# PolyU-IOR/HPR-LP-C

Hardware: AMD Instinct MI355X
Metric: HPR iterations/sec (FP64) (higher is better)
Workload: dtype f64

## Files before the change

### hpr-lp-c_amd/csrc/abi.cpp

```cpp
#include <algorithm>
#include <cmath>
#include <cstdlib>
#include <cstring>
#include <memory>
#include <mutex>
#include <iomanip>
#include <iostream>

#include "hprlp_amd.h"
#include "batch_prep.h"
#include "batched.h"
#include "env.h"
#include "dist.h"
#include "presolve.h"
#include "reorder.h"
#include "solver.h"
#include "many.h"
#include "values.h"
#include "version.h"

using namespace hprlp;

struct hprlp_solver {
    Solver s;
// ... 1242 lines not shown
    if (name == "x_temp") return {s.x_temp, s.n_loc, 'c'};
    if (name == "y") return {s.y, s.m_loc, 'r'};
    if (name == "last_y") return {s.last_y.p, s.m_loc, 'r'};
    if (name == "y_bar") return {s.y_bar, s.m_loc, 'r'};
    if (name == "y_obj") return {s.y_obj.p, s.m_loc, 'r'};
    if (name == "y_temp") return {s.y_temp.p, s.m_loc, 'r'};
    if (name == "AL") return {s.AL.p, s.m_loc, 'r'};
    if (name == "AU") return {s.AU.p, s.m_loc, 'r'};
    if (name == "l") return {s.l.p, s.n_loc, 'c'};
    if (name == "u") return {s.u.p, s.n_loc, 'c'};
    if (name == "c") return {s.c.p, s.n_loc, 'c'};
    if (name == "row_norm") return {s.row_norm.p, s.m_loc, 'r'};
    if (name == "col_norm") return {s.col_norm.p, s.n_loc, 'c'};
    if (name == "A_val") return {s.A.val.p, s.A.view.nnz, '-'};
    if (name == "AT_val") return {s.AT.val.p, s.AT.view.nnz, '-'};
    return {nullptr, -1, '-'};
}
const std::vector<int> *perm_of(const Solver &s, const VecRef &v) {
    if (v.kind == 'r' && !s.perm_r.empty()) return &s.perm_r;
    if (v.kind == 'c' && !s.perm_c.empty()) return &s.perm_c;
    return nullptr;
}
}

extern "C" long hprlp_solver_get_vector(hprlp_solver *h, const char *name, double *out, long cap) {
    GUARD_BEGIN
    VecRef v = find_vector(h->s, name ? name : "");
    if (v.n < 0) throw std::runtime_error(std::string("unknown vector name: ") + (name ? name : "(null)"));
    if (cap < v.n) throw std::runtime_error("output buffer too small");
    HIP_CHECK(hipStreamSynchronize(h->s.stream));
// ... 312 lines not shown
        d += t.n_pieces > 0 ? "tiled, piece form (k_tiled_part + k_tiled_finish, " + std::to_string(t.n_pieces) + " pieces)"
             : t.rem_cap == kPbRemCap ? "tiled, all-remainder form (k_pb_fused, grid " + std::to_string(t.grid) + ")"
                                      : "tiled, fused (k_tiled_fused, grid " + std::to_string(t.grid) + ")";
        d += ", " + std::to_string(t.nsb) + " super-blocks, " + std::to_string(M.tiled.n_steps) + " steps";
        if (t.R != kTileRows || t.T != kTileCols) d += " (" + std::to_string(t.R) + " rows, tiles of " + std::to_string(t.T) + " columns)";
        const double all = static_cast<double>(M.tiled.dense_entries) + static_cast<double>(M.tiled.n_rem);
        if (all > 0) d += ", " + std::to_string(static_cast<int>(100.0 * M.tiled.dense_entries / all + 0.5)) + " % of the entries in staged tiles";
        if (t.f_rk) d += ", source-side run tables";
        if (t.f_work) d += ", pre-pass work list of " + std::to_string(t.n_work) + " workgroups for " + std::to_string(t.n_groups) + " source groups";
        if (t.side_nblk > 0) d += ", long rows aside (" + std::to_string(t.side_nblk) + " blocks through the stream kernel)";
        return d;
    };
    std::string d = one("A", s.A) + "; " + one("A^T", s.AT);
    if (s.use_small && !s.comm) d += "; normal iterations in the single-workgroup kernel (k_small_iterations)";
    if (!s.perm_r.empty()) d += "; locality ordering applied at set-up";
    if (!s.env_at_setup.empty()) d += "; switches: " + s.env_at_setup;
    if (!s.env_ignored_at_setup.empty()) d += "; ignored without HPRLP_TEST_HOOKS=1: " + s.env_ignored_at_setup;
    std::snprintf(buf, static_cast<size_t>(cap), "%s", d.c_str());
    return static_cast<int>(d.size());
    GUARD_END(-1)
}

extern "C" int hprlp_form_select(const hprlp_form_facts *facts, const hprlp_form_hooks *hooks, hprlp_form_decision *out) {
    try {
        if (!facts || !out) throw std::runtime_error("bad arguments");
        const char *missing = "";
        if (!form_select(*facts, hooks ? *hooks : FormHooks(), out, &missing))
            throw std::runtime_error(std::string("the rules ask for a fact that the record marks as not measured: ") + missing);
        return 0;
    } catch (const std::exception &e) {
// ... 103 lines not shown
```

### hpr-lp-c_amd/csrc/env.cpp

```cpp
#include "env.h"

#include <cstdlib>
#include <cstring>
#include <stdexcept>

namespace hprlp {

static const EnvEntry kTable[] = {
    {"HPRLP_TEST_HOOKS", EnvKind::Integrator, "1: honour the test hooks below (tests/conftest.py and the tools/ scripts set it)"},
    {"HPRLP_TIMING", EnvKind::Integrator, "wall time of the set-up and solve phases on stderr"},
    {"HPRLP_NO_GRAPH", EnvKind::Integrator, "launch normal iterations eagerly instead of replaying hipGraphs (fall-back)"},
    {"HPRLP_NO_TILED", EnvKind::Integrator, "never build the column-tiled matrix copies: stream kernel everywhere (fall-back)"},
    {"HPRLP_NO_REORDER", EnvKind::Integrator, "no set-up time locality ordering of a large matrix"},
    {"HPRLP_NO_ALLOC_CACHE", EnvKind::Integrator, "do not keep freed device blocks for the next solver of the process"},
    {"HPRLP_DIST_TRANSPORT", EnvKind::Integrator, "shm: hprlp_dist_unique_id names a shared-memory segment (host-staged group of processes on one node) instead of RCCL ids"},
    {"HPRLP_NO_WARM_MODEL", EnvKind::Integrator, "the model constructors do NOT start the HIP runtime / device context / code objects (for a process that forks workers after building its models: a HIP context does not survive fork); the first solve pays for them as in the reference"},
    {"HPRLP_DIST_EXCHANGE", EnvKind::Hook, "sparse | allgather: force the multi-GPU exchange form (same value on every rank)"},
    {"HPRLP_NO_OVERLAP", EnvKind::Integrator, "multi-GPU: shards unsplit, exchange in line on the solver stream"},
    {"HPRLP_DIST_TIMEOUT_S", EnvKind::Integrator, "seconds a rank of the shared-memory transport waits for its peers before it fails (default 120)"},
    {"HPRLP_BATCH_CHUNK", EnvKind::Hook, "solve_batched with 64 or more problems: chunk width of the panels (default 64; narrower chunks map one chunk to each XCD -- measured slower, profiles/r03_tiled_decomposition.md section 6b)"},
    {"HPRLP_BATCH_GRID", EnvKind::Hook, "solve_batched: cap on the row blocks of the normal half-step kernels (read at every call; a small cap makes every workgroup's row loop wrap)"},
    {"HPRLP_BATCH_LAMBDA", EnvKind::Hook, "solve_batched: the batch's lambda_max from the caller (strtod; hand it over as a C99 hex float to keep every bit) instead of 1.01 x the power iteration's estimate (read at every call)"},
    {"HPRLP_COPY_PAUSE_US", EnvKind::Hook, "piece size and pause of the threaded copies of set-up (64 MB, 100 us)"},
    {"HPRLP_COPY_PIECE_MB", EnvKind::Hook, "piece size and pause of the threaded copies of set-up (64 MB, 100 us)"},
// ... 7 lines not shown
    {"HPRLP_HOST_TRANSPOSE", EnvKind::Hook, "build Aᵀ on the host / nonzero threshold of the device transpose (default 4 M)"},
    {"HPRLP_NO_BOUND_CODES", EnvKind::Hook, "the x-half always reads l[j] and u[j], the y-half AL[i] and AU[i] (default: one code byte per column / row says which of them is not a constant; an equality row reads one value)"},
    {"HPRLP_NO_FAR_PUSH", EnvKind::Hook, "always run the remainder pre-pass (k_far_products) instead of the hand-off from the producing half-step's epilogue"},
    {"HPRLP_NO_FAR_WORK", EnvKind::Hook, "the remainder pre-pass with one workgroup per source group also where one group holds several times the mean (default: a work list cuts heavy groups into chunks, tiled.h f_work)"},
    {"HPRLP_NO_PB_LONG_ROWS", EnvKind::Hook, "a matrix kept off the tiled forms for its long rows keeps the stream kernel also where its columns are not popular (default: all-remainder form, Solver::pb_fallback_wanted)"},
    {"HPRLP_NO_FUSED_NORMS", EnvKind::Hook, "the Ruiz row norms by their own passes instead of as a by-product of the preceding scaling pass (same bits)"},
    {"HPRLP_NO_LONG_SIDE", EnvKind::Hook, "a matrix with rows over 1024 entries keeps the stream kernel instead of being tiled with those rows kept aside"},
    {"HPRLP_NO_PB_FALLBACK", EnvKind::Hook, "unstructured large matrices keep the stream kernel instead of the tiled form without dense-tile requirement"},
    {"HPRLP_NO_PB_KERNEL", EnvKind::Hook, "run an all-remainder copy through k_tiled_fused's remainder steps instead of k_pb_fused (A/B)"},
    {"HPRLP_NO_REM2", EnvKind::Hook, "tiled build: no second remainder level"},
    {"HPRLP_NO_SETUP_OVERLAP", EnvKind::Hook, "set-up of a large model in line: no helper threads / copy streams for the value upload, the row blocks, A^T's row pointers and the model vectors (same bits either way)"},
    {"HPRLP_NO_SLAB_CUTS", EnvKind::Hook, "dense rows of a large matrix are not cut at the XCD eighths of the gathered vector (stream kernel)"},
    {"HPRLP_NO_SMALL", EnvKind::Hook, "do not use the single-workgroup kernel for Netlib-scale LPs"},
    {"HPRLP_NO_SMALL_POWER", EnvKind::Hook, "Netlib-scale LPs: power iteration by the regular kernels with the host test every 10th iteration (default: one launch of the single-workgroup kernel)"},
    {"HPRLP_NO_TILED_CR", EnvKind::Hook, "Curtis-Reid passes through the stream kernel also for matrices with a tiled copy (default: tiled kernel on a second value array of -log|a|)"},
    {"HPRLP_NT", EnvKind::Hook, "force default / nontemporal loads of the matrix in the stream kernel"},
    {"HPRLP_OVERLAP_COMM_FIRST", EnvKind::Hook, "tests only: with the in-process rank group, use RCCL's launch order (exchange enqueued before the local SpMV)"},
    {"HPRLP_PB_MIN_COLS", EnvKind::Hook, "gathered-vector length from which an unstructured matrix takes the all-remainder form (default 800 k columns, the crossover measured with k_pb_fused)"},
    {"HPRLP_PB_MIN_NNZ", EnvKind::Hook, "fewest entries for the all-remainder form"},
    {"HPRLP_PB_STAMPS", EnvKind::Hook, "developer build -DHPRLP_PB_PHASE_STAMPS=1: print k_pb_fused's phase times"},
    {"HPRLP_PIECES_ANYWAY", EnvKind::Hook, "attempt the tiled form although neighbouring rows gather from the same lines (<= 0.25 lines per entry) / keep the piece form although an XCD's rows gather from under 3 MB"},
    {"HPRLP_PRESOLVE_MAX_LINKS", EnvKind::Hook, "run one presolve stage alone / cut the chain after n links (tests, debugging)"},
    {"HPRLP_PRESOLVE_OFF", EnvKind::Hook, "switch presolve reductions / stages off (any subset; diagnostics)"},
    {"HPRLP_PRESOLVE_ONLY", EnvKind::Hook, "run one presolve stage alone / cut the chain after n links (tests, debugging)"},
    {"HPRLP_REORDER_CLUSTER", EnvKind::Hook, "knobs of the HOST reference path of the ordering (hprlp_locality_ordering): nodes per cluster, refinement sweeps, trimming percentage"},
    {"HPRLP_REORDER_HOST", EnvKind::Hook, "run the clustering of the locality ordering on the host (the reference form; default: on the device)"},
    {"HPRLP_REORDER_SWEEPS", EnvKind::Hook, "knobs of the HOST reference path of the ordering (hprlp_locality_ordering): nodes per cluster, refinement sweeps, trimming percentage"},
    {"HPRLP_REORDER_TRIM", EnvKind::Hook, "knobs of the HOST reference path of the ordering (hprlp_locality_ordering): nodes per cluster, refinement sweeps, trimming percentage"},
    {"HPRLP_SLACK_PIVOT", EnvKind::Hook, "pivot threshold of the costed slack-column substitution (default 0.5 of the row's largest entry)"},
    {"HPRLP_STORE_X", EnvKind::Hook, "every normal x-half reads and stores x (default for matrices with a tiled copy: inside a run of normal iterations x is rebuilt from x_hat and last_x by the next launch instead of travelling through memory)"},
// ... 52 lines not shown
```

### hpr-lp-c_amd/csrc/kernels.hip

```cpp
#include "kernels.h"

#include <algorithm>
#include <vector>
#include <cmath>
#include <type_traits>

namespace hprlp {

__device__ __forceinline__ double wave_sum(double v) {
#pragma unroll
    for (int off = 32; off > 0; off >>= 1) v += __shfl_xor(v, off, kWave);
    return v;
}

__device__ __forceinline__ double wave_max(double v) {
#pragma unroll
    for (int off = 32; off > 0; off >>= 1) v = fmax(v, __shfl_xor(v, off, kWave));
    return v;
}

template <int NACC, int NW, int NMAX = 0>
__device__ __forceinline__ void block_store_partials_in(double (&acc)[NACC], double *partials, int stride, double (*red)[NACC > 0 ? NACC : 1]) {
    const int wave = threadIdx.x >> 6, lane = threadIdx.x & 63;
#pragma unroll
// ... 210 lines not shown
    const int v = q == 0 ? a0 : (q == 1 ? a1 : (q == 2 ? a2 : a3));
    return __builtin_amdgcn_readlane(v, r & 63);
}

#ifndef HPRLP_PB_PHASE_STAMPS
#define HPRLP_PB_PHASE_STAMPS 0
#endif
#ifndef HPRLP_SWEEP_ED
#define HPRLP_SWEEP_ED 2
#define HPRLP_SWEEP_TD 1
#endif
#ifndef HPRLP_EPI_NT
#define HPRLP_EPI_NT 2
#endif

template <int ED, int TD, bool REP, bool STAMP = false, bool LOGTERM = false, int TC = kTileCols>
__device__ __forceinline__ void tiled_sweep(const TiledDev &t, int s0, int nst, int first, int count, const double *__restrict__ vec,
                                            int ncols, double *acc, double *ytile, int tid, unsigned long long *stamp = nullptr) {
    constexpr int NT = kTileThreads, R = kTileRows, K = kTileChunk;
    constexpr int TPT = TC / NT;
    static_assert(TC == kTileCols || TC == kTileColsNarrow, "tile width");
    typedef double d2_t __attribute__((ext_vector_type(2)));
    const int lane = tid & 63;
    auto sidx = [&](int i) { i = min(i, count - 1) + first; return s0 + (i < nst ? i : i - nst); };
    int seg = 0, lim = 0;
    int tc0 = 0, tc1 = 0, tc2 = 0, tc3 = 0, tb0 = 0, tb1 = 0, tb2 = 0, tb3 = 0, te0 = 0, te1 = 0, te2 = 0, te3 = 0;
    auto getstep = [&](int k, int &col0, int &eb, int &ee) {
        const int r = min(k, lim - 1) - seg;
        col0 = step_field(tc0, tc1, tc2, tc3, r);
        eb = step_field(tb0, tb1, tb2, tb3, r);
        ee = step_field(te0, te1, te2, te3, r);
    };
    struct Ent {
// ... 39 lines not shown
    };
    auto process = [&](const Ent &E, int k) {
        int col0, eb, ee_;
        getstep(k, col0, eb, ee_);
        if (K * tid < ee_ - eb) {
            const double v[K] = {E.va.x, E.va.y, E.vb.x, E.vb.y};
            const uint32_t c0 = E.i0, c1 = E.i1, c2 = E.i2;
            const uint32_t id[K] = {c0 & 0xffffffu, (c0 >> 24) | ((c1 & 0xffffu) << 8), (c1 >> 16) | ((c2 & 0xffu) << 16), c2 >> 8};
            uint32_t rw[K];
            double y[K];
#pragma unroll
            for (int k2 = 0; k2 < K; ++k2) {
                rw[k2] = id[k2] & (R - 1);
                y[k2] = ytile[id[k2] >> kTileRowBits];
            }
            double a[K];
#pragma unroll
            for (int k2 = 0; k2 < K; ++k2) a[k2] = acc[rw[k2]];
            double sk[K], pr[K];
#pragma unroll
            for (int k2 = 0; k2 < K; ++k2) pr[k2] = LOGTERM ? (v[k2] != v[k2] ? 0.0 : v[k2] - y[k2]) : v[k2] * y[k2];
            sk[0] = a[0] + pr[0];
#pragma unroll
            for (int k2 = 1; k2 < K; ++k2) sk[k2] = ((rw[k2] == rw[k2 - 1]) ? sk[k2 - 1] : a[k2]) + pr[k2];
#pragma unroll
            for (int k2 = 0; k2 < K; ++k2)
                if (k2 == K - 1 || rw[k2] != rw[k2 + 1]) acc[rw[k2]] = sk[k2];
        }
    };
    auto same_tile = [&](int k) {
// ... 1788 lines not shown
                         bool divide, hipStream_t s, double *next_max_norm) {
    if (M.rows <= 0 || M.nblk <= 0) return;
    if (next_max_norm) {
        if (row_first && divide) launch_scale_matrix_t<true, true, true>(M, rowvec, colvec_full, next_max_norm, s);
        else if (row_first && !divide) launch_scale_matrix_t<true, false, true>(M, rowvec, colvec_full, next_max_norm, s);
        else if (!row_first && divide) launch_scale_matrix_t<false, true, true>(M, rowvec, colvec_full, next_max_norm, s);
        else launch_scale_matrix_t<false, false, true>(M, rowvec, colvec_full, next_max_norm, s);
        return;
    }
    if (row_first && divide) launch_scale_matrix_t<true, true, false>(M, rowvec, colvec_full, nullptr, s);
    else if (row_first && !divide) launch_scale_matrix_t<true, false, false>(M, rowvec, colvec_full, nullptr, s);
    else if (!row_first && divide) launch_scale_matrix_t<false, true, false>(M, rowvec, colvec_full, nullptr, s);
    else launch_scale_matrix_t<false, false, false>(M, rowvec, colvec_full, nullptr, s);
}

__global__ void __launch_bounds__(kThreads) k_vec_scale(double *x, const double *s, int n, int divide) {
    const int i = blockIdx.x * kThreads + threadIdx.x;
    if (i < n) x[i] = divide ? x[i] / s[i] : x[i] * s[i];
}
void launch_vec_scale(double *x, const double *sv, int n, bool divide, hipStream_t s) {
    if (n <= 0) return;
    hipLaunchKernelGGL(k_vec_scale, dim3((n + kThreads - 1) / kThreads), dim3(kThreads), 0, s, x, sv, n, divide ? 1 : 0);
}

__global__ void __launch_bounds__(kThreads) k_vec_scal(double *x, double a, int n) {
    const int i = blockIdx.x * kThreads + threadIdx.x;
    if (i < n) x[i] = x[i] * a;
}
void launch_vec_scal(double *x, double a, int n, hipStream_t s) {
    if (n <= 0) return;
// ... 322 lines not shown
```

### hpr-lp-c_amd/csrc/solver.cpp

```cpp
#include "solver.h"
#include "env.h"

#include <algorithm>
#include <cmath>
#include <cstdio>
#include <cstdlib>
#include <cstring>
#include <functional>
#include <iomanip>
#include <iostream>
#include <limits>
#include <thread>

#include "dist.h"
#include "reorder.h"

namespace hprlp {

constexpr int kMaxGraphIters = 64;
constexpr int kDeviceStartRows = 1000000;
constexpr int kPowerBlockKey = -10;

struct RowCuts {
    std::vector<int> rows;
// ... 1097 lines not shown
        gsm2.alloc(static_cast<size_t>(m_pad));
        gsn2.alloc(static_cast<size_t>(n_pad));
        HIP_CHECK(hipMemsetAsync(gsm2.p, 0, sizeof(double) * m_pad, stream));
        HIP_CHECK(hipMemsetAsync(gsn2.p, 0, sizeof(double) * n_pad, stream));
    }
    double *gm = gsm.p, *gn = gsn.p, *gm_next = gsm2.p, *gn_next = gsn2.p;
    double *t1 = gm + row_off, *t2 = gn + col_off;
    double *t1n = fuse_norms ? gm_next + row_off : nullptr, *t2n = fuse_norms ? gn_next + col_off : nullptr;
    bool have_norms = false;
    const bool max_next = fuse_norms;
    launch_fill(row_norm.p, 1.0, m_loc, stream);
    launch_fill(col_norm.p, 1.0, n_loc, stream);
    norm_b_org = 1.0 + std::sqrt(bnorm_sq(this));
    norm_c_org = 1.0 + std::sqrt(reduce_sum_sq(c.p, n_loc));

    if (prm.use_CR_scaling) {
        HIP_CHECK(hipMemsetAsync(gsm.p, 0, sizeof(double) * m_pad, stream));
        HIP_CHECK(hipMemsetAsync(gsn.p, 0, sizeof(double) * n_pad, stream));
        finish_tiling();
        struct LogValues {
            DBuf<double> tile, far;
        } logA, logAT;
        const bool tiled_cr = env_get("HPRLP_NO_TILED_CR") == nullptr;
        auto log_values = [&](DeviceMatrix &M, LogValues &lv) {
            if (!tiled_cr || !cr_runs_tiled(M.view)) return;
            lv.tile.alloc(static_cast<size_t>(std::max<long>(M.tiled.n_tile, 1)));
            lv.far.alloc(static_cast<size_t>(std::max<long>(M.tiled.n_rem, 1)));
            launch_tiled_refresh_log(M.tiled, M.val.p, lv.tile.p, lv.far.p, stream);
        };
        log_values(A, logA);
        log_values(AT, logAT);
        for (int it = 0; it < 20; ++it) {
            launch_cr_log_update(A.view, gsn.p, t1, stream, logA.tile.p, logA.far.p);
            gather(gsm.p, true);
            launch_cr_log_update(AT.view, gsm.p, t2, stream, logAT.tile.p, logAT.far.p);
            gather(gsn.p, false);
        }
        if (logA.tile.p || logAT.tile.p) HIP_CHECK(hipStreamSynchronize(stream));
        launch_exp_clamp(t1, m_loc, stream);
        launch_exp_clamp(t2, n_loc, stream);
        gather(gsm.p, true);
        gather(gsn.p, false);
        launch_vec_scale(row_norm.p, t1, m_loc, true, stream);
        launch_vec_scale(col_norm.p, t2, n_loc, true, stream);
        launch_scale_matrix(A.view, t1, gsn.p, true, false, stream, max_next ? t1n : nullptr);
        launch_scale_matrix(AT.view, t2, gsm.p, false, false, stream, max_next ? t2n : nullptr);
        have_norms = max_next;
        launch_vec_scale(AL.p, t1, m_loc, false, stream);
        launch_vec_scale(AU.p, t1, m_loc, false, stream);
        launch_vec_scale(c.p, t2, n_loc, false, stream);
        launch_vec_scale(l.p, t2, n_loc, true, stream);
        launch_vec_scale(u.p, t2, n_loc, true, stream);
    }

    const int passes = (prm.use_Ruiz_scaling ? 10 : 0) + (prm.use_Pock_Chambolle_scaling ? 1 : 0);
    for (int it = 0; it < passes; ++it) {
        const int norm = (prm.use_Ruiz_scaling && it < 10) ? 99 : 1;
        if (have_norms) {
            std::swap(gm, gm_next);
            std::swap(gn, gn_next);
            t1 = gm + row_off, t2 = gn + col_off, t1n = gm_next + row_off, t2n = gn_next + col_off;
        } else {
            launch_row_norm(A.view, t1, norm, stream);
            launch_row_norm(AT.view, t2, norm, stream);
        }
        gather(gm, true);
        gather(gn, false);
        launch_vec_scale(row_norm.p, t1, m_loc, false, stream);
        launch_vec_scale(AL.p, t1, m_loc, true, stream);
        launch_vec_scale(AU.p, t1, m_loc, true, stream);
        launch_vec_scale(col_norm.p, t2, n_loc, false, stream);
        const bool next = fuse_norms && it + 1 < passes && it + 1 < 10;
        launch_scale_matrix(A.view, t1, gn, true, true, stream, next ? t1n : nullptr);
        launch_scale_matrix(AT.view, t2, gm, false, true, stream, next ? t2n : nullptr);
        have_norms = next;
        launch_vec_scale(c.p, t2, n_loc, true, stream);
        launch_vec_scale(l.p, t2, n_loc, false, stream);
        launch_vec_scale(u.p, t2, n_loc, false, stream);
    }

    if (prm.use_bc_scaling) {
        b_scale = 1.0 + std::sqrt(bnorm_sq(this));
        c_scale = 1.0 + std::sqrt(reduce_sum_sq(c.p, n_loc));
        const double bs = 1.0 / b_scale, cs = 1.0 / c_scale;
        launch_vec_scal(AU.p, bs, m_loc, stream);
        launch_vec_scal(AL.p, bs, m_loc, stream);
        launch_vec_scal(l.p, bs, n_loc, stream);
        launch_vec_scal(u.p, bs, n_loc, stream);
        launch_vec_scal(c.p, cs, n_loc, stream);
    } else {
        b_scale = 1.0;
        c_scale = 1.0;
    }
    norm_b = std::sqrt(bnorm_sq(this));
    norm_c = std::sqrt(reduce_sum_sq(c.p, n_loc));
    finish_tiling();
    A.refresh_tiled(stream);
    AT.refresh_tiled(stream);
    refresh_bound_codes();
    HIP_CHECK(hipMemsetAsync(gsm.p, 0, sizeof(double) * m_pad, stream));
    HIP_CHECK(hipMemsetAsync(gsn.p, 0, sizeof(double) * n_pad, stream));
    HIP_CHECK(hipStreamSynchronize(stream));
    scaling_time = time_since(t0);
    scaled = true;
}

SmallArgs Solver::small_args() const {
    return SmallArgs{m, n, A.view.nnz, A.view.rowptr, AT.view.rowptr, AT.view.val, small_ij.p, small_posA.p,
                     small_order_x.p, small_order_y.p, x.p, x_hat, y, l.p, u.p, c.p, last_x.p, AL.p, AU.p, last_y.p, ctrl.p};
}

bool Solver::small_power_wanted() const {
    const bool no_small_power = env_get("HPRLP_NO_SMALL_POWER") != nullptr;
    return use_small && !comm && !no_small_power;
}

void Solver::power_start(double *z) {
// ... 801 lines not shown
```

### hpr-lp-c_amd/csrc/solver.h

```cpp
#pragma once

#include <string>
#include <vector>

#include <functional>
#include <future>
#include <map>
#include <memory>

#include "common.h"
#include "env.h"
#include "dist.h"
#include "kernels.h"
#include "hpr_rules.h"
#include "form_select.h"

namespace hprlp {

struct TraceRow {
    int iter, restart_flag;
    double err_Rp, err_Rd, primal_obj, dual_obj, gap, kkt, sigma, current_gap, lambda_max;
};

struct DeviceMatrix {
// ... 81 lines not shown
    DBuf<unsigned char> lu_code;
    void refresh_bound_codes();
    DBuf<double> x, last_x, z_bar, last_y, y_obj, y_temp;
    DBuf<double> gy, gxh, gxb, gyb, gxt, gsn, gsm;
    double *y = nullptr, *x_hat = nullptr, *x_bar = nullptr, *y_bar = nullptr, *x_temp = nullptr;
    DBuf<double> sm1, sn1;
    DBuf<Ctrl> ctrl;
    DBuf<double> scal;
    HBuf<double> scal_h;
    DBuf<double> part_x, part_y, part_r, part_v;
    int stride_x = 0, stride_y = 0;

    double b_scale = 1, c_scale = 1, norm_b = 0, norm_c = 0, norm_b_org = 1, norm_c_org = 1;
    double sigma = 1.0, lambda_max = 1.0;
    double setup_time = 0, scaling_time = 0, power_time = 0;
    double fetch_enqueue_s = 0, fetch_wait_s = 0;
    long fetches = 0;
    int power_iters = 0;
    bool use_graph = true;
    bool use_small = false;
    int max_row_A = 0, max_row_AT = 0;
    DBuf<int> small_order_x, small_order_y;
    DBuf<int> small_ij, small_posA;

    Detection detect;
    DBuf<double> ray_prev_x, ray_prev_y, ray_d, ray_y, ray_part;
    bool ray_have_prev = false;
    Certificate cert;
    void ray_begin();
    bool ray_test();
// ... 100 lines not shown
```

### hpr-lp-c_amd/csrc/tiled.h

```cpp
#pragma once

#include <hip/hip_runtime.h>

#include <cstdint>
#include <vector>

#include "common.h"

namespace hprlp {

constexpr int kTileThreads = 512;
constexpr int kTileRows = 8192;
constexpr int kTileCols = 2048;
constexpr int kTileColsNarrow = 1024;
constexpr int kTileChunk = 4;
constexpr int kTileStepCap = kTileThreads * kTileChunk;
constexpr int kTileRemK = 4;
constexpr int kTileRemCap = (kTileThreads - 4) * kTileRemK;
constexpr int kTileRemRun = 16;
#ifndef HPRLP_PB_REM_K
#define HPRLP_PB_REM_K 8
#endif
constexpr int kPbRemK = HPRLP_PB_REM_K;
constexpr int kPbRemCap = kTileThreads * kPbRemK;
// ... 131 lines not shown

void tiled_host_check(int rows, int cols, const int *rp, const int *ci, int R, int T, double min_dense, long out[6]);

void compact_without_rows(long nnz, int rows, const int *rp_dev, const int *rp_c_dev, const int *col_dev, int *col_c, int *map_c, hipStream_t s);

struct DeviceTiled {
    DBuf<int> sb_ptr, sb_mid, tperm, rperm, rcol;
    DBuf<TileStep> steps;
    DBuf<uint32_t> tidx;
    DBuf<uint32_t> tidx3;
    DBuf<uint16_t> rrow;
    DBuf<double> tval;
    DBuf<double> P, f_val;
    DBuf<uint32_t> rq;
    DBuf<int> f_gptr, f_pos, f_perm;
    DBuf<int> f_rptr, f_rk, f_rp;
    DBuf<int4> f_work;
    DBuf<uint16_t> f_lcol;
    TiledDev view;
    long n_tile = 0, n_rem = 0;
    double rem_top_share = 0.0;
    long dense_entries = 0, padding = 0;
    int n_steps = 0;
    void upload(const TiledHost &h, int R = kTileRows, int T = kTileCols, int rem_cap = kTileRemCap);
    void pack_indices(hipStream_t s);
    void build_far(int cols, hipStream_t s, int G = kTileRows);
    void finish_schedule(hipStream_t s);
    int rot_period = 0;
    DBuf<double> parts;
    DBuf<int> piece_ptr, slot_ptr;
// ... 2 lines not shown
    DBuf<unsigned long long> wgtimes;
    DBuf<int4> side_blk, side_long;
    DBuf<int> side_rows;
    DBuf<double> side_partial, base;
    void set_side(int rows, const int *rowptr_host, const std::vector<int> &long_rows);
    void compose_perms(const int *map_dev, hipStream_t s);
    void dump_wgtimes() const;
    DBuf<int4> segs;
    bool build_on_device(int rows, int cols, long nnz, const int *rowptr, const int *col, int min_rows,
                         double min_dense_fraction, hipStream_t s, int R = kTileRows, int T = kTileCols, int rem_cap = kTileRemCap);
    void compare_with(const TiledHost &h) const;
};

void launch_tiled_refresh(const DeviceTiled &t, const double *csr_val, hipStream_t s);
void launch_tiled_refresh_log(const DeviceTiled &t, const double *csr_val, double *tval_log, double *fval_log, hipStream_t s);

}
```

### hpr-lp-c_amd/csrc/tiled_build.hip

```cpp
#include <algorithm>
#include <functional>
#include <cstdlib>
#include <hipcub/hipcub.hpp>

#include <vector>

#include "common.h"
#include "env.h"
#include "kernels.h"
#include "tiled.h"

namespace hprlp {

namespace {

constexpr int K = kTileChunk;
constexpr int kRowBits = kTileRowBits;

__device__ __forceinline__ int row_of_entry(const int *__restrict__ rowptr, int rows, int k) {
    int lo = 0, hi = rows;
    while (hi - lo > 1) {
        const int mid = lo + ((hi - lo) >> 1);
        if (rowptr[mid] <= k) lo = mid;
        else hi = mid;
// ... 630 lines not shown
    const int step = static_cast<int>(skey[i] >> 32), e = static_cast<int>(skey[i] & 0xffffffffu);
    const int slot = p_sorted[i] - steps[step].e_begin;
    rq[i] = (static_cast<uint32_t>(slot) << 16) | static_cast<uint32_t>(rrow[e]);
}

__global__ void __launch_bounds__(kThreads) k_far_key_f(int n, int G, const int *__restrict__ e_of_p, const int *__restrict__ rcol,
                                                       unsigned long long *__restrict__ key, int *__restrict__ val) {
    const int p = blockIdx.x * kThreads + threadIdx.x;
    if (p >= n) return;
    key[p] = (static_cast<unsigned long long>(rcol[e_of_p[p]] / G) << 32) | static_cast<unsigned long long>(p);
    val[p] = e_of_p[p];
}

__global__ void __launch_bounds__(kThreads) k_far_fill_f(int n, int G, const unsigned long long *__restrict__ skey, const int *__restrict__ e_sorted,
                                                        const int *__restrict__ rcol, const int *__restrict__ rperm, int *__restrict__ f_pos,
                                                        uint16_t *__restrict__ f_lcol, int *__restrict__ f_perm) {
    const int f = blockIdx.x * kThreads + threadIdx.x;
    if (f >= n) return;
    const int g = static_cast<int>(skey[f] >> 32), e = e_sorted[f];
    f_pos[f] = static_cast<int>(skey[f] & 0xffffffffu);
    f_lcol[f] = static_cast<uint16_t>(rcol[e] - g * G);
    f_perm[f] = rperm[e];
}

__global__ void __launch_bounds__(kThreads) k_far_gptr(int ngroups, int n, const unsigned long long *__restrict__ skey, int *__restrict__ gptr) {
    const int g = blockIdx.x * kThreads + threadIdx.x;
    if (g > ngroups) return;
    int lo = 0, hi = n;
    while (lo < hi) {
        const int mid = lo + ((hi - lo) >> 1);
        if (static_cast<int>(skey[mid] >> 32) < g) lo = mid + 1;
        else hi = mid;
    }
    gptr[g] = lo;
}

__global__ void __launch_bounds__(kThreads) k_far_run_flags(int n, const unsigned long long *__restrict__ skey, const int *__restrict__ f_pos,
// ... 35 lines not shown
int bits_for(long v) {
    int b = 1;
    while ((1L << b) <= v) ++b;
    return b;
}

}

void DeviceTiled::build_far(int cols, hipStream_t s, int G) {
    static_assert(kFarGroup <= 65536 && kTileRemCap <= 65536 && kTileRows <= 65536, "16-bit local columns, slots and rows");
    if (G < 64 || G > kFarGroup) throw std::runtime_error("remainder lists: unsupported source-group size");
    view.G = G;
    view.P = nullptr;
    view.rq = nullptr;
    view.n_groups = 0;
    if (!view.valid || n_rem <= 0) {
        rcol.release(); rrow.release(); rperm.release();
        return;
    }
    const int n = static_cast<int>(n_rem), nsb = view.nsb;
    const int ngroups = (cols + G - 1) / G;
    DBuf<int> step_of(static_cast<size_t>(n)), sb_of(static_cast<size_t>(n));
    const char *no2 = env_get("HPRLP_NO_REM2");
    hipLaunchKernelGGL(k_far_step_of, dim3(nsb), dim3(kThreads), 0, s, nsb, sb_ptr.p, sb_mid.p, steps.p, rrow.p, step_of.p, sb_of.p, !(no2 && no2[0] == '1'));
    if (env_get("HPRLP_TIMING")) {
        std::vector<TileStep> hs(static_cast<size_t>(n_steps));
        std::vector<int> hp(static_cast<size_t>(nsb) + 1), hm(static_cast<size_t>(nsb));
        HIP_CHECK(hipStreamSynchronize(s));
        steps.download(hs.data(), hs.size());
        sb_ptr.download(hp.data(), hp.size());
        sb_mid.download(hm.data(), hm.size());
        long rem_steps = 0, marked = 0, most = 0;
        for (int sb = 0; sb < nsb; ++sb) {
            most = std::max<long>(most, hp[sb + 1] - hm[sb]);
            for (int q = hm[sb]; q < hp[sb + 1]; ++q) {
                ++rem_steps;
                marked += hs[q].col0 != 0;
            }
        }
        std::fprintf(stderr, "[timing]   remainder: %ld steps (most in one super-block: %ld), %ld with a long run of one row\n", rem_steps, most, marked);
    }
    DBuf<unsigned long long> kin(static_cast<size_t>(n)), kout(static_cast<size_t>(n));
    DBuf<int> vin(static_cast<size_t>(n)), e_of_p(static_cast<size_t>(n));
    hipLaunchKernelGGL(k_far_key_p, dim3(grid_for(n)), dim3(kThreads), 0, s, n, G, sb_of.p, rcol.p, kin.p, vin.p);
    sort_pairs(kin, kout, vin, e_of_p, n, 32 + bits_for(nsb), s);
    sb_of.release();
    DBuf<int> p_sorted(static_cast<size_t>(n));
    hipLaunchKernelGGL(k_far_key_q, dim3(grid_for(n)), dim3(kThreads), 0, s, n, step_of.p, e_of_p.p, kin.p, vin.p);
    sort_pairs(kin, kout, vin, p_sorted, n, 32 + bits_for(n_steps), s);
    rq.alloc_zero(static_cast<size_t>(n) + 8);
    hipLaunchKernelGGL(k_far_fill_q, dim3(grid_for(n)), dim3(kThreads), 0, s, n, kout.p, p_sorted.p, steps.p, rrow.p, rq.p);
    HIP_CHECK(hipStreamSynchronize(s));
    step_of.release();
    hipLaunchKernelGGL(k_far_key_f, dim3(grid_for(n)), dim3(kThreads), 0, s, n, G, e_of_p.p, rcol.p, kin.p, vin.p);
    sort_pairs(kin, kout, vin, p_sorted, n, 32 + bits_for(ngroups), s);
    f_pos.alloc_zero(static_cast<size_t>(n) + 8);
    f_lcol.alloc_zero(static_cast<size_t>(n) + 8);
    f_perm.alloc(static_cast<size_t>(n) + 8);
    f_val.alloc_zero(static_cast<size_t>(n) + 8);
    f_gptr.alloc(static_cast<size_t>(ngroups) + 1);
    hipLaunchKernelGGL(k_far_fill_f, dim3(grid_for(n)), dim3(kThreads), 0, s, n, G, kout.p, p_sorted.p, rcol.p, rperm.p, f_pos.p, f_lcol.p, f_perm.p);
    hipLaunchKernelGGL(k_far_gptr, dim3(grid_for(ngroups + 1)), dim3(kThreads), 0, s, ngroups, n, kout.p, f_gptr.p);
    P.alloc_zero(static_cast<size_t>(n) + 8);
    HIP_CHECK(hipStreamSynchronize(s));
    {
        std::vector<int> gp(static_cast<size_t>(ngroups) + 1);
        f_gptr.download(gp.data(), gp.size());
        const long cap = std::max<long>(kFarWorkMin, kFarWorkOverMean * static_cast<long>(n) / std::max(ngroups, 1));
        int heaviest = 0;
        for (int g = 0; g < ngroups; ++g) heaviest = std::max(heaviest, gp[g + 1] - gp[g]);
        {
            std::vector<int> sz(static_cast<size_t>(ngroups));
            for (int g = 0; g < ngroups; ++g) sz[g] = gp[g + 1] - gp[g];
            const int k = std::max(1, std::min(ngroups, static_cast<int>((2L << 20) / (8L * G))));
            std::nth_element(sz.begin(), sz.begin() + (k - 1), sz.end(), std::greater<int>());
            long top = 0;
            for (int g = 0; g < k; ++g) top += sz[g];
            rem_top_share = static_cast<double>(top) / static_cast<double>(n);
        }
// ... 233 lines not shown
```

Baseline: 770.3.

## Run Ruiz scaling passes directly on tiled matrix copies, write back once

When A and A^T both use the fused tiled form, the ten Ruiz scaling passes now scale the tiled copies' own value arrays in a tiled sweep kernel (plus a remainder kernel) and compute next row norms there, instead of scaling the CSR arrays. The CSR values are written back once after the last pass, which avoids scaling CSR and then refreshing the tiled copies. The change adds per-entry row/column index arrays for the remainder and moves finish_tiling earlier. This affects set-up time; iteration throughput should be unaffected unless rounding differences change the scaled matrix.

Result: no change. 768.0 (-0.3%).

```diff
diff --git a/hpr-lp-c_amd/csrc/abi.cpp b/hpr-lp-c_amd/csrc/abi.cpp
--- a/hpr-lp-c_amd/csrc/abi.cpp
+++ b/hpr-lp-c_amd/csrc/abi.cpp
@@ -1280,6 +1280,10 @@
     if (name == "col_norm") return {s.col_norm.p, s.n_loc, 'c'};
     if (name == "A_val") return {s.A.val.p, s.A.view.nnz, '-'};
     if (name == "AT_val") return {s.AT.val.p, s.AT.view.nnz, '-'};
+    if (name == "A_tval") return {s.A.tiled.tval.p, s.A.view.tiled.valid ? s.A.tiled.n_tile : 0, '-'};
+    if (name == "A_fval") return {s.A.tiled.f_val.p, s.A.view.tiled.valid && s.A.tiled.f_val.p ? s.A.tiled.n_rem : 0, '-'};
+    if (name == "AT_tval") return {s.AT.tiled.tval.p, s.AT.view.tiled.valid ? s.AT.tiled.n_tile : 0, '-'};
+    if (name == "AT_fval") return {s.AT.tiled.f_val.p, s.AT.view.tiled.valid && s.AT.tiled.f_val.p ? s.AT.tiled.n_rem : 0, '-'};
     return {nullptr, -1, '-'};
 }
 const std::vector<int> *perm_of(const Solver &s, const VecRef &v) {
@@ -1622,6 +1626,7 @@
     std::string d = one("A", s.A) + "; " + one("A^T", s.AT);
     if (s.use_small && !s.comm) d += "; normal iterations in the single-workgroup kernel (k_small_iterations)";
     if (!s.perm_r.empty()) d += "; locality ordering applied at set-up";
+    if (s.tiled_scaling_passes > 0) d += "; scaling: " + std::to_string(s.tiled_scaling_passes) + " Ruiz passes on the tiled copies";
     if (!s.env_at_setup.empty()) d += "; switches: " + s.env_at_setup;
     if (!s.env_ignored_at_setup.empty()) d += "; ignored without HPRLP_TEST_HOOKS=1: " + s.env_ignored_at_setup;
     std::snprintf(buf, static_cast<size_t>(cap), "%s", d.c_str());
diff --git a/hpr-lp-c_amd/csrc/env.cpp b/hpr-lp-c_amd/csrc/env.cpp
--- a/hpr-lp-c_amd/csrc/env.cpp
+++ b/hpr-lp-c_amd/csrc/env.cpp
@@ -45,6 +45,7 @@
     {"HPRLP_NO_SMALL", EnvKind::Hook, "do not use the single-workgroup kernel for Netlib-scale LPs"},
     {"HPRLP_NO_SMALL_POWER", EnvKind::Hook, "Netlib-scale LPs: power iteration by the regular kernels with the host test every 10th iteration (default: one launch of the single-workgroup kernel)"},
     {"HPRLP_NO_TILED_CR", EnvKind::Hook, "Curtis-Reid passes through the stream kernel also for matrices with a tiled copy (default: tiled kernel on a second value array of -log|a|)"},
+    {"HPRLP_NO_TILED_SCALING", EnvKind::Hook, "Ruiz passes over the CSR value arrays also for matrices whose A and A^T both run the fused tiled form (default: on the tiled copies' own values, written back to the CSR arrays once)"},
     {"HPRLP_NT", EnvKind::Hook, "force default / nontemporal loads of the matrix in the stream kernel"},
     {"HPRLP_OVERLAP_COMM_FIRST", EnvKind::Hook, "tests only: with the in-process rank group, use RCCL's launch order (exchange enqueued before the local SpMV)"},
     {"HPRLP_PB_MIN_COLS", EnvKind::Hook, "gathered-vector length from which an unstructured matrix takes the all-remainder form (default 800 k columns, the crossover measured with k_pb_fused)"},
diff --git a/hpr-lp-c_amd/csrc/kernels.hip b/hpr-lp-c_amd/csrc/kernels.hip
--- a/hpr-lp-c_amd/csrc/kernels.hip
+++ b/hpr-lp-c_amd/csrc/kernels.hip
@@ -248,9 +248,16 @@
 #define HPRLP_EPI_NT 2
 #endif
 
-template <int ED, int TD, bool REP, bool STAMP = false, bool LOGTERM = false, int TC = kTileCols>
+struct SweepScale {
+    double *rmax = nullptr;
+    double *tval = nullptr;
+    bool row_first = true, divide = true;
+};
+
+template <int ED, int TD, bool REP, bool STAMP = false, bool LOGTERM = false, int TC = kTileCols, bool SCALE = false>
 __device__ __forceinline__ void tiled_sweep(const TiledDev &t, int s0, int nst, int first, int count, const double *__restrict__ vec,
-                                            int ncols, double *acc, double *ytile, int tid, unsigned long long *stamp = nullptr) {
+                                            int ncols, double *acc, double *ytile, int tid, unsigned long long *stamp = nullptr,
+                                            const SweepScale sc = SweepScale()) {
     constexpr int NT = kTileThreads, R = kTileRows, K = kTileChunk;
     constexpr int TPT = TC / NT;
     static_assert(TC == kTileCols || TC == kTileColsNarrow, "tile width");
@@ -320,6 +327,28 @@
                 rw[k2] = id[k2] & (R - 1);
                 y[k2] = ytile[id[k2] >> kTileRowBits];
             }
+            if constexpr (SCALE) {
+                double nv[K], mx[K];
+#pragma unroll
+                for (int k2 = 0; k2 < K; ++k2) {
+                    const double rv = acc[rw[k2]];
+                    const double d0 = sc.row_first ? rv : y[k2], d1 = sc.row_first ? y[k2] : rv;
+                    nv[k2] = sc.divide ? (v[k2] / d0) / d1 : (v[k2] * d0) * d1;
+                    mx[k2] = nv[k2] == nv[k2] ? fabs(nv[k2]) : 0.0;
+                }
+                d2_t o0, o1;
+                o0.x = nv[0]; o0.y = nv[1]; o1.x = nv[2]; o1.y = nv[3];
+                d2_t *dst = reinterpret_cast<d2_t *>(sc.tval + eb + K * tid);
+                __builtin_nontemporal_store(o0, dst);
+                __builtin_nontemporal_store(o1, dst + 1);
+#pragma unroll
+                for (int k2 = 1; k2 < K; ++k2)
+                    if (rw[k2] == rw[k2 - 1] && mx[k2] < mx[k2 - 1]) mx[k2] = mx[k2 - 1];
+#pragma unroll
+                for (int k2 = 0; k2 < K; ++k2)
+                    if ((k2 == K - 1 || rw[k2] != rw[k2 + 1]) && sc.rmax[rw[k2]] < mx[k2]) sc.rmax[rw[k2]] = mx[k2];
+                return;
+            }
             double a[K];
 #pragma unroll
             for (int k2 = 0; k2 < K; ++k2) a[k2] = acc[rw[k2]];
@@ -2138,6 +2167,114 @@
     else launch_scale_matrix_t<false, false, false>(M, rowvec, colvec_full, nullptr, s);
 }
 
+__device__ __forceinline__ double scale_entry_rt(double v, double rv, double cv, bool row_first, bool divide) {
+    const double d0 = row_first ? rv : cv, d1 = row_first ? cv : rv;
+    return divide ? (v / d0) / d1 : (v * d0) * d1;
+}
+
+__global__ void __launch_bounds__(kThreads) k_far_scale(long n, double *__restrict__ f_val, const int *__restrict__ f_row,
+                                                       const int *__restrict__ f_col, const int *__restrict__ f_pos,
+                                                       const double *__restrict__ rowvec, const double *__restrict__ colvec,
+                                                       double *__restrict__ P, bool row_first, bool divide) {
+    const long i = static_cast<long>(blockIdx.x) * kThreads + threadIdx.x;
+    if (i >= n) return;
+    const double nv = scale_entry_rt(f_val[i], rowvec[f_row[i]], colvec[f_col[i]], row_first, divide);
+    f_val[i] = nv;
+    P[f_pos[i]] = nv;
+}
+
+template <bool NARROW>
+__global__ void __launch_bounds__(kTileThreads, 2) k_tiled_scale(TiledDev t, int rows, int ncols, double *tval,
+                                                                const double *__restrict__ rowvec, const double *__restrict__ colvec,
+                                                                double *next_norm, bool row_first, bool divide) {
+    constexpr int NT = kTileThreads;
+    __shared__ double rfac[kTileRows];
+    __shared__ double rmax[kTileRows];
+    __shared__ __attribute__((aligned(16))) double ytile[kTileCols];
+    const int tid = threadIdx.x;
+    const int R = t.R;
+    const int per = t.per, slots = gridDim.x / 8, slot = blockIdx.x / 8;
+    for (int q = slot; q < per; q += slots) {
+        const int sb = (blockIdx.x % 8) * per + q;
+        if (sb >= t.nsb) break;
+        const int s0 = t.sb_ptr[sb], smid = t.sb_mid[sb], s1 = t.sb_ptr[sb + 1];
+        const int r0 = sb * R;
+        const int nr = min(R, rows - r0);
+        lds_barrier();
+        for (int i = tid; i < R; i += NT) {
+            rfac[i] = i < nr ? rowvec[r0 + i] : 1.0;
+            rmax[i] = 0.0;
+        }
+        SweepScale sc;
+        sc.rmax = rmax;
+        sc.tval = tval;
+        sc.row_first = row_first;
+        sc.divide = divide;
+        if (s0 < smid)
+            tiled_sweep<HPRLP_SWEEP_ED, HPRLP_SWEEP_TD, false, false, false, NARROW ? kTileColsNarrow : kTileCols, true>(
+                t, s0, smid - s0, t.steps[s0].rot, smid - s0, colvec, ncols, rfac, ytile, tid, nullptr, sc);
+        if (!next_norm) continue;
+        lds_barrier();
+        for (int st = smid; st < s1; ++st) {
+            const int eb = t.steps[st].e_begin, cnt = t.steps[st].e_end - eb;
+            for (int i = tid; i < cnt; i += NT) {
+                const uint32_t code = t.rq[eb + i];
+                const double a = fabs(t.P[eb + (code >> 16)]);
+                if (a > 0.0)
+                    atomicMax(reinterpret_cast<unsigned long long *>(rmax + (code & 0xffffu)), static_cast<unsigned long long>(__double_as_longlong(a)));
+            }
+        }
+        lds_barrier();
+        for (int i = tid; i < nr; i += NT) next_norm[r0 + i] = norm_result(rmax[i]);
+    }
+}
+
+__global__ void __launch_bounds__(kThreads) k_tiled_writeback(long n, const int *__restrict__ perm, const double *__restrict__ src,
+                                                             double *__restrict__ csr_val) {
+    const long i = static_cast<long>(blockIdx.x) * kThreads + threadIdx.x;
+    if (i < n) {
+        const int p = perm[i];
+        if (p >= 0) csr_val[p] = src[i];
+    }
+}
+
+template <bool NARROW>
+static void launch_tiled_scale_t(const DeviceTiled &t, int grid, int rows, int cols, const double *rowvec, const double *colvec_full,
+                                 bool row_first, bool divide, double *next_norm, hipStream_t s) {
+    hipLaunchKernelGGL(k_tiled_scale<NARROW>, dim3(grid), dim3(kTileThreads), 0, s, t.view, rows, cols, t.tval.p, rowvec,
+                       colvec_full, next_norm, row_first, divide);
+}
+
+void launch_tiled_scale(const DeviceTiled &t, int rows, int cols, const double *rowvec, const double *colvec_full, bool row_first,
+                        bool divide, hipStream_t s, double *next_max_norm) {
+    if (rows <= 0 || !t.view.valid) return;
+    if (t.n_rem > 0) {
+        if (!t.f_row.p || !t.f_col.p || !t.view.f_pos || !t.view.P || !t.view.rq)
+            throw std::runtime_error("tiled scaling pass: the remainder's rows and columns have been released");
+        hipLaunchKernelGGL(k_far_scale, dim3(static_cast<unsigned>((t.n_rem + kThreads - 1) / kThreads)), dim3(kThreads), 0, s, t.n_rem, t.f_val.p,
+                           t.f_row.p, t.f_col.p, t.view.f_pos, rowvec, colvec_full, t.view.P, row_first, divide);
+    }
+    static const int cus_per_xcd = [] {
+        int dev = 0, cus = 256;
+        HIP_CHECK(hipGetDevice(&dev));
+        HIP_CHECK(hipDeviceGetAttribute(&cus, hipDeviceAttributeMultiprocessorCount, dev));
+        return std::max(1, cus / 8);
+    }();
+    const int grid = 8 * std::min(t.view.per, cus_per_xcd);
+    const bool narrow = t.view.T == kTileColsNarrow;
+    if (narrow) launch_tiled_scale_t<true>(t, grid, rows, cols, rowvec, colvec_full, row_first, divide, next_max_norm, s);
+    else launch_tiled_scale_t<false>(t, grid, rows, cols, rowvec, colvec_full, row_first, divide, next_max_norm, s);
+}
+
+void launch_tiled_writeback(const DeviceTiled &t, double *csr_val, hipStream_t s) {
+    if (t.n_tile > 0)
+        hipLaunchKernelGGL(k_tiled_writeback, dim3(static_cast<unsigned>((t.n_tile + kThreads - 1) / kThreads)), dim3(kThreads), 0, s,
+                           t.n_tile, t.tperm.p, t.tval.p, csr_val);
+    if (t.n_rem > 0 && t.f_val.p)
+        hipLaunchKernelGGL(k_tiled_writeback, dim3(static_cast<unsigned>((t.n_rem + kThreads - 1) / kThreads)), dim3(kThreads), 0, s,
+                           t.n_rem, t.f_perm.p, t.f_val.p, csr_val);
+}
+
 __global__ void __launch_bounds__(kThreads) k_vec_scale(double *x, const double *s, int n, int divide) {
     const int i = blockIdx.x * kThreads + threadIdx.x;
     if (i < n) x[i] = divide ? x[i] / s[i] : x[i] * s[i];
diff --git a/hpr-lp-c_amd/csrc/solver.cpp b/hpr-lp-c_amd/csrc/solver.cpp
--- a/hpr-lp-c_amd/csrc/solver.cpp
+++ b/hpr-lp-c_amd/csrc/solver.cpp
@@ -1135,6 +1135,25 @@
     norm_b_org = 1.0 + std::sqrt(bnorm_sq(this));
     norm_c_org = 1.0 + std::sqrt(reduce_sum_sq(c.p, n_loc));
 
+    auto scales_tiled = [](const DeviceMatrix &M) {
+        const TiledDev &t = M.view.tiled;
+        return t.valid && t.n_pieces == 0 && t.side_nblk == 0 && t.rem_cap != kPbRemCap && (M.tiled.n_rem == 0 || (M.tiled.f_row.p && M.tiled.f_col.p));
+    };
+    tiled_scaling_passes = 0;
+    bool on_copies = false;
+    if (prm.use_Ruiz_scaling && fuse_norms && !comm && env_get("HPRLP_NO_TILED_SCALING") == nullptr) {
+        finish_tiling();
+        on_copies = scales_tiled(A) && scales_tiled(AT);
+        if (on_copies && scaled) {
+            A.refresh_tiled(stream);
+            AT.refresh_tiled(stream);
+        }
+    }
+    auto scale_pass = [&](DeviceMatrix &M, const double *rowvec, const double *colvec_full, bool row_first, bool divide, bool on_copy, double *next_norm) {
+        if (on_copy) launch_tiled_scale(M.tiled, M.view.rows, M.view.cols, rowvec, colvec_full, row_first, divide, stream, next_norm);
+        else launch_scale_matrix(M.view, rowvec, colvec_full, row_first, divide, stream, next_norm);
+    };
+
     if (prm.use_CR_scaling) {
         HIP_CHECK(hipMemsetAsync(gsm.p, 0, sizeof(double) * m_pad, stream));
         HIP_CHECK(hipMemsetAsync(gsn.p, 0, sizeof(double) * n_pad, stream));
@@ -1164,8 +1183,8 @@
         gather(gsn.p, false);
         launch_vec_scale(row_norm.p, t1, m_loc, true, stream);
         launch_vec_scale(col_norm.p, t2, n_loc, true, stream);
-        launch_scale_matrix(A.view, t1, gsn.p, true, false, stream, max_next ? t1n : nullptr);
-        launch_scale_matrix(AT.view, t2, gsm.p, false, false, stream, max_next ? t2n : nullptr);
+        scale_pass(A, t1, gsn.p, true, false, on_copies, max_next ? t1n : nullptr);
+        scale_pass(AT, t2, gsm.p, false, false, on_copies, max_next ? t2n : nullptr);
         have_norms = max_next;
         launch_vec_scale(AL.p, t1, m_loc, false, stream);
         launch_vec_scale(AU.p, t1, m_loc, false, stream);
@@ -1177,6 +1196,7 @@
     const int passes = (prm.use_Ruiz_scaling ? 10 : 0) + (prm.use_Pock_Chambolle_scaling ? 1 : 0);
     for (int it = 0; it < passes; ++it) {
         const int norm = (prm.use_Ruiz_scaling && it < 10) ? 99 : 1;
+        const bool on_copy = on_copies && it < 10;
         if (have_norms) {
             std::swap(gm, gm_next);
             std::swap(gn, gn_next);
@@ -1192,9 +1212,16 @@
         launch_vec_scale(AU.p, t1, m_loc, true, stream);
         launch_vec_scale(col_norm.p, t2, n_loc, false, stream);
         const bool next = fuse_norms && it + 1 < passes && it + 1 < 10;
-        launch_scale_matrix(A.view, t1, gn, true, true, stream, next ? t1n : nullptr);
-        launch_scale_matrix(AT.view, t2, gm, false, true, stream, next ? t2n : nullptr);
+        scale_pass(A, t1, gn, true, true, on_copy, next ? t1n : nullptr);
+        scale_pass(AT, t2, gm, false, true, on_copy, next ? t2n : nullptr);
         have_norms = next;
+        if (on_copy) {
+            ++tiled_scaling_passes;
+            if (it == 9) {
+                launch_tiled_writeback(A.tiled, A.val.p, stream);
+                launch_tiled_writeback(AT.tiled, AT.val.p, stream);
+            }
+        }
         launch_vec_scale(c.p, t2, n_loc, true, stream);
         launch_vec_scale(l.p, t2, n_loc, false, stream);
         launch_vec_scale(u.p, t2, n_loc, false, stream);
@@ -1222,6 +1249,9 @@
     HIP_CHECK(hipMemsetAsync(gsm.p, 0, sizeof(double) * m_pad, stream));
     HIP_CHECK(hipMemsetAsync(gsn.p, 0, sizeof(double) * n_pad, stream));
     HIP_CHECK(hipStreamSynchronize(stream));
+    invalidate_far();
+    A.tiled.f_row.release(); A.tiled.f_col.release();
+    AT.tiled.f_row.release(); AT.tiled.f_col.release();
     scaling_time = time_since(t0);
     scaled = true;
 }
diff --git a/hpr-lp-c_amd/csrc/solver.h b/hpr-lp-c_amd/csrc/solver.h
--- a/hpr-lp-c_amd/csrc/solver.h
+++ b/hpr-lp-c_amd/csrc/solver.h
@@ -119,6 +119,7 @@
     double b_scale = 1, c_scale = 1, norm_b = 0, norm_c = 0, norm_b_org = 1, norm_c_org = 1;
     double sigma = 1.0, lambda_max = 1.0;
     double setup_time = 0, scaling_time = 0, power_time = 0;
+    int tiled_scaling_passes = 0;
     double fetch_enqueue_s = 0, fetch_wait_s = 0;
     long fetches = 0;
     int power_iters = 0;
diff --git a/hpr-lp-c_amd/csrc/tiled.h b/hpr-lp-c_amd/csrc/tiled.h
--- a/hpr-lp-c_amd/csrc/tiled.h
+++ b/hpr-lp-c_amd/csrc/tiled.h
@@ -169,6 +169,7 @@
     DBuf<double> P, f_val;
     DBuf<uint32_t> rq;
     DBuf<int> f_gptr, f_pos, f_perm;
+    DBuf<int> f_row, f_col;
     DBuf<int> f_rptr, f_rk, f_rp;
     DBuf<int4> f_work;
     DBuf<uint16_t> f_lcol;
@@ -201,5 +202,8 @@
 
 void launch_tiled_refresh(const DeviceTiled &t, const double *csr_val, hipStream_t s);
 void launch_tiled_refresh_log(const DeviceTiled &t, const double *csr_val, double *tval_log, double *fval_log, hipStream_t s);
+void launch_tiled_scale(const DeviceTiled &t, int rows, int cols, const double *rowvec, const double *colvec_full, bool row_first,
+                        bool divide, hipStream_t s, double *next_max_norm);
+void launch_tiled_writeback(const DeviceTiled &t, double *csr_val, hipStream_t s);
 
 }
diff --git a/hpr-lp-c_amd/csrc/tiled_build.hip b/hpr-lp-c_amd/csrc/tiled_build.hip
--- a/hpr-lp-c_amd/csrc/tiled_build.hip
+++ b/hpr-lp-c_amd/csrc/tiled_build.hip
@@ -668,13 +668,19 @@
 
 __global__ void __launch_bounds__(kThreads) k_far_fill_f(int n, int G, const unsigned long long *__restrict__ skey, const int *__restrict__ e_sorted,
                                                         const int *__restrict__ rcol, const int *__restrict__ rperm, int *__restrict__ f_pos,
-                                                        uint16_t *__restrict__ f_lcol, int *__restrict__ f_perm) {
+                                                        uint16_t *__restrict__ f_lcol, int *__restrict__ f_perm,
+                                                        const int *__restrict__ sb_of, const uint16_t *__restrict__ rrow, int R,
+                                                        int *__restrict__ f_row, int *__restrict__ f_col) {
     const int f = blockIdx.x * kThreads + threadIdx.x;
     if (f >= n) return;
     const int g = static_cast<int>(skey[f] >> 32), e = e_sorted[f];
     f_pos[f] = static_cast<int>(skey[f] & 0xffffffffu);
     f_lcol[f] = static_cast<uint16_t>(rcol[e] - g * G);
     f_perm[f] = rperm[e];
+    if (f_row) {
+        f_row[f] = sb_of[e] * R + static_cast<int>(rrow[e]);
+        f_col[f] = rcol[e];
+    }
 }
 
 __global__ void __launch_bounds__(kThreads) k_far_gptr(int ngroups, int n, const unsigned long long *__restrict__ skey, int *__restrict__ gptr) {
@@ -740,6 +746,7 @@
     view.P = nullptr;
     view.rq = nullptr;
     view.n_groups = 0;
+    f_row.release(); f_col.release();
     if (!view.valid || n_rem <= 0) {
         rcol.release(); rrow.release(); rperm.release();
         return;
@@ -770,7 +777,6 @@
     DBuf<int> vin(static_cast<size_t>(n)), e_of_p(static_cast<size_t>(n));
     hipLaunchKernelGGL(k_far_key_p, dim3(grid_for(n)), dim3(kThreads), 0, s, n, G, sb_of.p, rcol.p, kin.p, vin.p);
     sort_pairs(kin, kout, vin, e_of_p, n, 32 + bits_for(nsb), s);
-    sb_of.release();
     DBuf<int> p_sorted(static_cast<size_t>(n));
     hipLaunchKernelGGL(k_far_key_q, dim3(grid_for(n)), dim3(kThreads), 0, s, n, step_of.p, e_of_p.p, kin.p, vin.p);
     sort_pairs(kin, kout, vin, p_sorted, n, 32 + bits_for(n_steps), s);
@@ -785,10 +791,16 @@
     f_perm.alloc(static_cast<size_t>(n) + 8);
     f_val.alloc_zero(static_cast<size_t>(n) + 8);
     f_gptr.alloc(static_cast<size_t>(ngroups) + 1);
-    hipLaunchKernelGGL(k_far_fill_f, dim3(grid_for(n)), dim3(kThreads), 0, s, n, G, kout.p, p_sorted.p, rcol.p, rperm.p, f_pos.p, f_lcol.p, f_perm.p);
+    if (view.rem_cap != kPbRemCap) {
+        f_row.alloc(static_cast<size_t>(n));
+        f_col.alloc(static_cast<size_t>(n));
+    }
+    hipLaunchKernelGGL(k_far_fill_f, dim3(grid_for(n)), dim3(kThreads), 0, s, n, G, kout.p, p_sorted.p, rcol.p, rperm.p, f_pos.p, f_lcol.p, f_perm.p,
+                       sb_of.p, rrow.p, view.R, f_row.p, f_col.p);
     hipLaunchKernelGGL(k_far_gptr, dim3(grid_for(ngroups + 1)), dim3(kThreads), 0, s, ngroups, n, kout.p, f_gptr.p);
     P.alloc_zero(static_cast<size_t>(n) + 8);
     HIP_CHECK(hipStreamSynchronize(s));
+    sb_of.release();
     {
         std::vector<int> gp(static_cast<size_t>(ngroups) + 1);
         f_gptr.download(gp.data(), gp.size());
```
